# mit-acl/rl_collision_avoidance

Hardware: AMD Instinct MI355X
Metric: agent-steps/sec (env.step) at 4 agents x 8192 worlds per GPU (higher is better)
Workload: dtype f64

## Files before the change

__graft_entry__.py:

```python
import os
import sys

ROOT = os.path.dirname(os.path.abspath(__file__))
if ROOT not in sys.path:
    sys.path.insert(0, ROOT)


def build() -> None:
    from rl_collision_avoidance_amd import build as hip_build
    path = hip_build.build(verbose=True)
    assert os.path.exists(path)
    try:
        for kind in (1, 2, 3, 4):
            hip_build.build_ulp_fault(kind)
    except Exception as exc:
        print("warning: development variant not built (%s); the tests that need it build it themselves" % exc)
    try:
        hip_build.build_crowd_dev()
    except Exception as exc:
        print("warning: crowd development variant not built (%s); tests/test_gpu_crowd.py builds it itself" % exc)
    try:
        hip_build.build_plain_dist()
    except Exception as exc:
        print("warning: plain-distance development variant not built (%s); tests/test_gpu_relay_trim.py builds it itself" % exc)
    from oracle import c_oracle
    c_oracle.build()
    import rl_collision_avoidance_amd
    from rl_collision_avoidance_amd import _lib
    handle = _lib.lib()
    for name, _, _ in _lib.SYMBOLS:
        getattr(handle, name)
    print("build ok:", path)


def smoke() -> None:
    import numpy as np
    import torch
    from oracle import c_oracle as co
    from rl_collision_avoidance_amd.batched_env import BatchedCollisionAvoidanceEnv

    assert torch.cuda.is_available(), "smoke() needs cuda:0"
    W, N, seed = 256, 4, 17
    env = BatchedCollisionAvoidanceEnv(W, device="cuda:0", seed=seed)
    env.reset()
    ocfg, ogen = co.default_cfg(N), co.default_gen(N, N, pool_size=int(env.cfg.gen_pool_size))
    st = co.State.empty(W, N)
    ep = np.zeros(W, np.uint32)
    co.generate(ocfg, ogen, seed, st, ep)
    rng = np.random.default_rng(seed)
    for t in range(40):
        acts = rng.integers(0, 11, size=(W, N)).astype(np.int32)
        obs, rew, done, go = env.step_autoreset(torch.from_numpy(acts).cuda())
        oobs, orew, odone, ogo = co.step_autoreset(ocfg, ogen, seed, st, ep, acts)
        assert np.array_equal(done.cpu().numpy(), odone) and np.array_equal(go.cpu().numpy(), ogo)
        d = np.abs(obs.cpu().numpy() - oobs)
        d[..., 3] = np.minimum(d[..., 3], np.abs(d[..., 3] - 2 * np.pi))
        assert d.max() <= 1e-5
        assert np.abs(rew.cpu().numpy() - orew).max() <= 1e-5
    fl = env.get_state()[2].cpu().numpy().view(np.uint32)
    assert np.array_equal(fl, st.flags)
    acts16 = rng.integers(0, 11, size=(16, W, N)).astype(np.int32)
    slots = env.new_step_slots(16, packed=True)
    pk_all, go_all = env.step_autoreset_packed(torch.from_numpy(acts16).cuda(), slots)
    wdt = env.obs_width
    for k in range(16):
        oobs, orew, odone, ogo = co.step_autoreset(ocfg, ogen, seed, st, ep, acts16[k])
        pk = pk_all[k].cpu().numpy()
        d = np.abs(pk[..., :wdt] - oobs)
        d[..., 3] = np.minimum(d[..., 3], np.abs(d[..., 3] - 2 * np.pi))
        assert d.max() <= 1e-5 and np.abs(pk[..., wdt] - orew).max() <= 1e-5, k
        assert np.array_equal(pk[..., wdt + 1].astype(np.uint8), odone) and np.array_equal(go_all[k].cpu().numpy(), ogo), k
    assert np.array_equal(env.get_state()[2].cpu().numpy().view(np.uint32), st.flags)
    obs = torch.from_numpy(np.ascontiguousarray(pk[..., :wdt])).cuda()
    from rl_collision_avoidance_amd.ga3c.network import NetworkVP_rnn
    from rl_collision_avoidance_amd.ga3c.policy_kernel import FusedPolicy
    net = NetworkVP_rnn(env.config).to("cuda:0")
    view = obs.view(W * N, -1)[:, 1:]
# ... 44 lines not shown
```

rl_collision_avoidance_amd/build.py:

```python
from __future__ import annotations

import os
import shutil
import subprocess

PKG_DIR = os.path.dirname(os.path.abspath(__file__))
ROOT = os.path.dirname(PKG_DIR)
CSRC = os.path.join(PKG_DIR, "csrc")
LIB_PATH = os.path.join(PKG_DIR, "libcavoid_hip.so")
SOURCES = [os.path.join(CSRC, "cavoid_capi.hip"), os.path.join(CSRC, "cavoid_multistep.hip"), os.path.join(CSRC, "cavoid_rvo.hip"),
           os.path.join(CSRC, "cavoid_relay.hip"), os.path.join(CSRC, "cavoid_quad.hip"), os.path.join(CSRC, "cavoid_rollout_capi.hip"),
           os.path.join(CSRC, "cavoid_policy_capi.hip"), os.path.join(CSRC, "cavoid_comm_capi.hip"), os.path.join(CSRC, "cavoid_actor.hip"),
           os.path.join(CSRC, "cavoid_actor_rvo.hip"), os.path.join(CSRC, "cavoid_actor_frozen.hip"), os.path.join(CSRC, "cavoid_crowd.hip"),
           os.path.join(CSRC, "cavoid_policy_ws.hip"), os.path.join(CSRC, "cavoid_policy_train_ring.hip"),
           os.path.join(CSRC, "cavoid_policy_wsring.hip"), os.path.join(CSRC, "cavoid_crowd_push.hip"), os.path.join(CSRC, "cavoid_crowd_rvo.hip"),
           os.path.join(CSRC, "cavoid_crowd_actor.hip")]
HEADERS = {
    "cavoid_capi.hip": ["cavoid_kernels.hpp", "cavoid_launch.hpp", "cavoid_host.hpp", "cavoid_crowd.hpp", "cavoid_crowd_rvo.hpp"],
    "cavoid_multistep.hip": ["cavoid_kernels.hpp", "cavoid_launch.hpp", "cavoid_host.hpp"],
    "cavoid_rvo.hip": ["cavoid_kernels.hpp", "cavoid_launch.hpp", "cavoid_host.hpp"],
    "cavoid_relay.hip": ["cavoid_kernels.hpp", "cavoid_relay.hpp", "cavoid_launch.hpp", "cavoid_host.hpp"],
    "cavoid_quad.hip": ["cavoid_kernels.hpp", "cavoid_quad.hpp", "cavoid_launch.hpp", "cavoid_host.hpp"],
    "cavoid_rollout_capi.hip": ["cavoid_rollout.hpp", "cavoid_rollout_host.hpp", "cavoid_host.hpp"],
    "cavoid_policy_capi.hip": ["cavoid_policy.hpp", "cavoid_policy_split.hpp", "cavoid_policy_split8.hpp", "cavoid_policy_crowd.hpp", "cavoid_policy_host.hpp",
# ... 145 lines not shown
    out = variant_path("crowd2")
    if os.path.exists(out):
        return out
    build()
    objs = _compile_objects([], "", False, verbose)
    jobs, swap = [], {}
    for name in ("cavoid_capi.hip", "cavoid_multistep.hip", "cavoid_crowd.hip", "cavoid_crowd_rvo.hip"):
        src = os.path.join(CSRC, name)
        obj = os.path.join(OBJ_DIR, name.replace(".hip", ".crowd2.o"))
        jobs.append([hipcc()] + FLAGS + EXTRA_FLAGS.get(name, []) + ["-DCAVOID_DEV_CROWD_FROM_N=2", "-DCAVOID_DEV_ONLY_N", "-c", src, "-o", obj])
        swap[os.path.join(OBJ_DIR, name.replace(".hip", ".o"))] = obj
    if verbose:
        for j in jobs:
            print(" ".join(j), flush=True)
    with ThreadPoolExecutor(max_workers=len(jobs)) as pool:
        list(pool.map(subprocess.check_call, jobs))
    for old in glob.glob(os.path.join(FAULT_DIR, "libcavoid_hip_crowd2-*.so")):
        os.remove(old)
    tmp = out + ".tmp"
    _link([swap.get(o, o) for o in objs], tmp, verbose)
    os.replace(tmp, out)
    return out


def build_plain_dist(verbose: bool = False) -> str:
    import glob
    from concurrent.futures import ThreadPoolExecutor
    out = variant_path("plaindist")
    if os.path.exists(out):
        return out
    build()
    objs = _compile_objects([], "", False, verbose)
    jobs, swap = [], {}
    for name in ("cavoid_capi.hip", "cavoid_multistep.hip", "cavoid_rvo.hip", "cavoid_relay.hip"):
        src = os.path.join(CSRC, name)
        obj = os.path.join(OBJ_DIR, name.replace(".hip", ".plaindist.o"))
        jobs.append([hipcc()] + FLAGS + EXTRA_FLAGS.get(name, []) +
                    ["-DCAVOID_MIRROR_DIST=0", "-DCAVOID_RELAY_ROLE_ARGS=0", "-DCAVOID_DEV_ONLY_N", "-DCAVOID_DEV_ENV_NS=3,4,5,6,10",
                     "-DCAVOID_DEV_RELAY_NS=3,4,5,6", "-c", src, "-o", obj])
        swap[os.path.join(OBJ_DIR, name.replace(".hip", ".o"))] = obj
    if verbose:
        for j in jobs:
            print(" ".join(j), flush=True)
    with ThreadPoolExecutor(max_workers=len(jobs)) as pool:
        list(pool.map(subprocess.check_call, jobs))
    for old in glob.glob(os.path.join(FAULT_DIR, "libcavoid_hip_plaindist-*.so")):
        os.remove(old)
    tmp = out + ".tmp"
    _link([swap.get(o, o) for o in objs], tmp, verbose)
    os.replace(tmp, out)
    return out


if __name__ == "__main__":
    import sys
    if "--trace" in sys.argv:
        print(build_trace(verbose=True))
    elif "--plain-dist" in sys.argv:
        print(build_plain_dist(verbose=True))
    elif "--crowd-dev" in sys.argv:
        print(build_crowd_dev(verbose=True))
    elif "--ulp-faults" in sys.argv:
        for kind in (1, 2, 3, 4):
            print(build_ulp_fault(kind, verbose=True))
    else:
        print(build(force=True, verbose=True))
```

rl_collision_avoidance_amd/csrc/cavoid_kernels.hpp:

```cpp
#pragma once
#include <hip/hip_runtime.h>
#include <stdint.h>

#include "cavoid.h"

namespace cavoid {

#ifdef CAVOID_TRACE
__device__ unsigned long long *g_trace = nullptr;
#define CAVOID_STAMP(k)                                                                \
    do {                                                                               \
        if (lane == 0 && g_trace) g_trace[wave * 16 + (k)] = (unsigned long long)clock64(); \
    } while (0)
#else
#define CAVOID_STAMP(k) do { } while (0)
#endif

#define CAVOID_RARE(x) __builtin_expect(!!(x), 0)
#ifndef CAVOID_SKIP
#define CAVOID_SKIP 0
#endif

constexpr double kPi = 3.14159265358979323846;
constexpr int kTileMaxAgents = 16;
// ... 15 lines not shown
    int32_t max_other, width, sort_method, dynamics, actions_fp32, timeout_enabled, num_actions;
    int32_t gen_mode, rvo_enabled;
    uint32_t pool_epoch;
    int32_t pool_size;
    int32_t ahead;
    int32_t prefetch_pool;
    int32_t tile_rows;
    int32_t wpw;
    int32_t rvo_lds_floats;
    int32_t park_floats;
    int32_t evaluate_mode;
    int32_t stream_obs;
    uint32_t switches;
    uint32_t seed_lo, seed_hi;
    int64_t num_worlds, world_offset;
    const double *action_table;
};

enum : uint32_t {
    kSwSkipDonePairs = 1u,
    kSwExactGap = 2u,
    kSwIndexTie = 4u,
    kSwWrapClosed = 8u,
};
struct KState {
    double *px, *py, *heading, *t_rem;
    float *gx, *gy, *radius, *pref, *speed;
    uint32_t *flags;
    uint32_t *episode;
};

struct alignas(64) PoolRec {
    double px, py, heading, t_rem;
    float gx, gy, radius, pref;
    uint32_t flags;
    uint32_t pad[3];
};
static_assert(sizeof(PoolRec) == 64, "pool record must be one 64-byte line");

struct KIO {
    PoolRec *pool_out;
    const int32_t *actions;
    const float *cont;
    const uint8_t *mask;
    float *obs;
    float *rew;
    uint8_t *done;
    uint8_t *game_over;
    int64_t action_stride;
    int64_t out_step_stride;
    int32_t n_steps;
    int32_t obs_stride;
    int32_t packed;
    uint32_t *ahead_hi;
};

__device__ __forceinline__ double wrap_closed_fixup(double a, uint32_t switches) {
    if (CAVOID_RARE(switches & kSwWrapClosed)) a = a == -kPi ? kPi : a;
    return a;
}
__device__ __forceinline__ double wrap_angle(double a, uint32_t switches) {
    a = a >= kPi ? a - 2.0 * kPi : a;
    a = a < -kPi ? a + 2.0 * kPi : a;
    if (CAVOID_RARE(__ballot(a >= kPi || a < -kPi) != 0ull)) {
        while (a >= kPi) a -= 2.0 * kPi;
        while (a < -kPi) a += 2.0 * kPi;
    }
    return wrap_closed_fixup(a, switches);
}
__device__ __forceinline__ double wrap_once(double h, uint32_t switches) {
    h = h >= kPi ? h - 2.0 * kPi : h;
    h = h < -kPi ? h + 2.0 * kPi : h;
    return wrap_closed_fixup(h, switches);
}

__device__ __forceinline__ void wave_lds_sync() {
    __builtin_amdgcn_fence(__ATOMIC_RELEASE, "wavefront");
    __builtin_amdgcn_wave_barrier();
    __builtin_amdgcn_fence(__ATOMIC_ACQUIRE, "wavefront");
}

struct U4 { uint32_t x, y, z, w; };
__device__ __forceinline__ U4 philox4x32(uint32_t c0, uint32_t c1, uint32_t c2, uint32_t c3, uint32_t k0, uint32_t k1) {
#pragma unroll
    for (int r = 0; r < 10; ++r) {
        const uint64_t p0 = (uint64_t)0xD2511F53u * c0, p1 = (uint64_t)0xCD9E8D57u * c2;
        const uint32_t n0 = (uint32_t)(p1 >> 32) ^ c1 ^ k0, n1 = (uint32_t)p1;
        const uint32_t n2 = (uint32_t)(p0 >> 32) ^ c3 ^ k1, n3 = (uint32_t)p0;
        c0 = n0; c1 = n1; c2 = n2; c3 = n3;
        k0 += 0x9E3779B9u; k1 += 0xBB67AE85u;
    }
    return U4{c0, c1, c2, c3};
}
__device__ __forceinline__ double u01(uint32_t r) { return (double)(r >> 8) * (1.0 / 16777216.0); }

struct Agent {
    double px, py, heading, t_rem, vx, vy;
    float gx, gy, radius, pref, speed;
    uint32_t flags;
};

struct alignas(16) StageRec { double px, py; float vxf, vyf, r, pad; };
static_assert(sizeof(StageRec) == 32, "two 16-byte reads per neighbour");
constexpr int kRingDoubleFromN = 6;
__host__ __device__ constexpr int lds_floats_block() { return 64 * 2; }
__host__ __device__ constexpr int lds_floats_fixed(int n) { return (n >= kRingDoubleFromN ? 128 : 64) * (int)(sizeof(StageRec) / sizeof(float)); }
// ... 1491 lines not shown
```

rl_collision_avoidance_amd/csrc/cavoid_launch.hpp:

```cpp
#pragma once
#include <hip/hip_runtime.h>
#include <hip/hip_ext.h>

#include <type_traits>

#include "cavoid.h"
#include "cavoid_host.hpp"
#include "cavoid_kernels.hpp"

struct cavoid_env {
    int device = 0;
    int64_t W = 0, A = 0, world_offset = 0;
    cavoid_cfg cfg{};
    cavoid::KCfg k{};
    cavoid::KState st{};
    cavoid::PoolRec *pool = nullptr;
    uint32_t *pool_episode = nullptr;
    int64_t pool_size = 0;
    int ahead_R = 0;
    uint32_t *ahead_hi[2] = {nullptr, nullptr};
    int ahead_cur = 0;
    int ahead_budget = 0;
    bool ahead_primed = false;
    bool ahead_always = false;
    int64_t ahead_refills = 0;
    int relay_topup_nc = -1;
    size_t relay_topup_lds = 0;
    bool relay_topup_fits = false;
    void *slab = nullptr;
    void *pool_slab = nullptr;
    double *d_actions = nullptr;
    int waves_per_block = 4;
    int grid = 0;
    int pipeline = 2;
    int relay_consumers = 3;
    int latency_mode = 0;
    int quad = -1;
    int prefetch_single = 0;
    int last_form = CAVOID_FORM_NONE;
    int last_relay_consumers = 0;
    hipEvent_t ev0 = nullptr, ev1 = nullptr;
};


namespace cavoid {

template <int... Ns>
struct NList {};
#ifdef CAVOID_DEV_ONLY_N
#ifndef CAVOID_DEV_ENV_NS
#define CAVOID_DEV_ENV_NS 4, 10
#endif
#ifndef CAVOID_DEV_RELAY_NS
#define CAVOID_DEV_RELAY_NS 4
#endif
using EnvNs = NList<CAVOID_DEV_ENV_NS>;
using RelayNs = NList<CAVOID_DEV_RELAY_NS>;
using QuadNs = NList<4>;
#else
using EnvNs = NList<1, 2, 3, 4, 5, 6, 7, 8, 9, 10, 11, 12, 13, 14, 15, 16>;
using RelayNs = NList<1, 2, 3, 4, 5, 6>;
using QuadNs = NList<2, 3, 4, 5, 6, 10>;
#endif

#ifdef CAVOID_DEV_CROWD_FROM_N
constexpr int kCrowdFromN = CAVOID_DEV_CROWD_FROM_N;
#else
constexpr int kCrowdFromN = kTileMaxAgents + 1;
#endif
static inline bool crowd_form(int max_agents) { return max_agents >= kCrowdFromN; }

template <int... Ns, class F>
static inline int dispatch_n(int n, NList<Ns...>, F &&f) {
    int rc = CAVOID_EUNSUPPORTED;
    (void)((n == Ns ? (rc = f(std::integral_constant<int, Ns>{}), true) : false) || ...);
    return rc;
}

template <class K, class... Args>
static inline void launch_kernel(K kernel, dim3 grid, dim3 block, size_t lds, hipStream_t s, hipEvent_t ev_start, hipEvent_t ev_stop,
                                 const Args &...args) {
// ... 86 lines not shown
```

rl_collision_avoidance_amd/csrc/cavoid_relay.hip:

```cpp
#include "cavoid_launch.hpp"
#include "cavoid_relay.hpp"

using namespace cavoid;

constexpr int kRelayMaxDevices = 64;
template <int N>
static int relay_allow_lds() {
    static bool allowed[kRelayMaxDevices] = {};
    int dev = 0;
    HIP_TRY(hipGetDevice(&dev));
    const bool cached = dev >= 0 && dev < kRelayMaxDevices;
    if (cached && allowed[dev]) return CAVOID_OK;
    if (hipFuncSetAttribute(reinterpret_cast<const void *>(env_relay_kernel<N>), hipFuncAttributeMaxDynamicSharedMemorySize, (int)kRelayLdsLimit) != hipSuccess) {
        (void)hipGetLastError();
        return CAVOID_EUNSUPPORTED;
    }
    if (cached) allowed[dev] = true;
    return CAVOID_OK;
}

struct RelayShape {
    int nc = 0;
    size_t lds = 0;
    bool topup = false;
};
template <int N>
static int relay_shape_n(cavoid_env *e, int tile_floats, bool want_topup, RelayShape &sh) {
    int nc = e->relay_consumers;
    while (nc > 1 && relay_lds_fixed_bytes<N>() + (size_t)nc * tile_floats * sizeof(float) > kRelayLdsLimit) --nc;
    const size_t lds = relay_lds_fixed_bytes<N>() + (size_t)nc * tile_floats * sizeof(float);
    if (lds > kRelayLdsLimit || (nc < 2 && e->relay_consumers >= 2)) return CAVOID_EUNSUPPORTED;
    if (lds > 65536) {
        const int rc_opt = relay_allow_lds<N>();
        if (rc_opt != CAVOID_OK) return rc_opt;
    }
    sh.nc = nc;
    sh.lds = lds;
    sh.topup = false;
    if (want_topup && e->k.gen_mode == 0) {
        if (e->relay_topup_nc != nc || e->relay_topup_lds != lds) {
            int blocks = 0;
            if (hipOccupancyMaxActiveBlocksPerMultiprocessor(&blocks, reinterpret_cast<const void *>(env_relay_kernel<N>), 64 * (4 + nc), lds) != hipSuccess) {
                (void)hipGetLastError();
                blocks = 0;
            }
            e->relay_topup_nc = nc;
            e->relay_topup_lds = lds;
            e->relay_topup_fits = blocks >= 2;
        }
        sh.topup = e->relay_topup_fits;
    }
    return CAVOID_OK;
}
static int relay_shape(cavoid_env *e, const KIO &io, bool want_topup, RelayShape &sh) {
    const KCfg &k = e->k;
    if (k.rvo_enabled || k.pool_size <= 0 || !io.obs || !io.actions || io.cont) return CAVOID_EUNSUPPORTED;
    if (k.switches & kSwSkipDonePairs) return CAVOID_EUNSUPPORTED;
    const int64_t tiles = (e->W + k.wpw - 1) / k.wpw;
    if (tiles > 512) return CAVOID_EUNSUPPORTED;
    if (e->cfg.max_agents > kRelayMaxAgents) return CAVOID_EUNSUPPORTED;
    const int row = io.obs_stride;
    const int tile_floats = (k.tile_rows * row + 3) & ~3;
    if (k.tile_rows < k.wpw * e->cfg.max_agents) return CAVOID_EUNSUPPORTED;
    return dispatch_n(e->cfg.max_agents, RelayNs{}, [&](auto n) -> int { return relay_shape_n<decltype(n)::value>(e, tile_floats, want_topup, sh); });
}

static bool relay_wants_topup(const cavoid_env *e, hipStream_t s) {
    if (e->ahead_R <= 0 || e->ahead_always || e->k.gen_mode != 0) return false;
    hipStreamCaptureStatus cap = hipStreamCaptureStatusNone;
    (void)hipStreamIsCapturing(s, &cap);
    return cap == hipStreamCaptureStatusNone;
}

bool cavoid_relay_takes_topup(cavoid_env *e, const KIO &io, hipStream_t s) {
    RelayShape sh;
    return relay_wants_topup(e, s) && relay_shape(e, io, true, sh) == CAVOID_OK && sh.topup;
}

int cavoid_launch_relay(cavoid_env *e, const KIO &io, hipStream_t s, hipEvent_t ev_start, hipEvent_t ev_stop) {
    RelayShape sh;
    const int rc_shape = relay_shape(e, io, io.ahead_hi != nullptr, sh);
    if (rc_shape != CAVOID_OK) return rc_shape;
    if ((io.ahead_hi != nullptr) != sh.topup) return CAVOID_EINVAL;
    const int64_t tiles = (e->W + e->k.wpw - 1) / e->k.wpw;
    const dim3 grid((unsigned)tiles), block(64 * (3 + sh.nc + (sh.topup ? 1 : 0)));
    const int rc = dispatch_n(e->cfg.max_agents, RelayNs{}, [&](auto n) -> int {
        launch_kernel(env_relay_kernel<decltype(n)::value>, grid, block, sh.lds, s, ev_start, ev_stop, e->k, e->st, e->pool, io);
        return CAVOID_OK;
    });
    if (rc != CAVOID_OK) return rc;
    HIP_TRY(hipGetLastError());
    return note_form(e, CAVOID_OK, CAVOID_FORM_RELAY, sh.nc);
}

#ifdef CAVOID_TRACE
int cavoid_debug_trace_relay(unsigned long long *dev_ptr) { return set_trace(dev_ptr); }
#endif
```

rl_collision_avoidance_amd/csrc/cavoid_relay.hpp:

```cpp
#pragma once
#include <cstddef>
#include <type_traits>

#include "cavoid_kernels.hpp"

namespace cavoid {

constexpr int kRelayMaxAgents = 6;
template <int N>
__host__ __device__ constexpr int relay_ring() { return N <= 5 ? 8 : 4; }
constexpr size_t kRelayLdsLimit = 80 * 1024;
constexpr int kRelayActRing = 64;
constexpr int kRelayActAhead = 48;
constexpr int kRelayEvq = 8;
constexpr int kRelayTopupMaxN = 5;

struct RelaySeq {
    int spec;
    int stage;
    int res;
    int fin;
    int act;
    int ev;
    int nxt;
    int cons[kRelayMaxConsumers];
    int cfin[kRelayMaxConsumers];
    int coop[2];
    int kernarg[2];
    int tile_id;
};
static_assert(sizeof(RelaySeq) % 16 == 0, "the event queue behind it holds 64-bit masks; the tiles further on are read 16 bytes at a time");
struct RelayTent { double px[64], py[64], vx[64], vy[64], heading[64]; float r[64], gx[64], gy[64], pref[64]; uint32_t flags[64]; };
struct RelayRes { uint32_t flags[64], ctl[64]; float rew[64]; };
struct RelayNxt { double px[64], py[64], heading[64], t_rem[64]; float gx[64], gy[64], radius[64], pref[64]; uint32_t flags[64]; };
#ifndef CAVOID_RELAY_ORDER
#define CAVOID_RELAY_ORDER 0x6432150
#endif
#ifndef CAVOID_RELAY_PRIO_D
#define CAVOID_RELAY_PRIO_D 3
#endif
#ifndef CAVOID_RELAY_PRIO_P
#define CAVOID_RELAY_PRIO_P 3
#endif
#ifndef CAVOID_RELAY_PRIO_L
#define CAVOID_RELAY_PRIO_L 0
#endif
#ifndef CAVOID_RELAY_PRIO_C
#define CAVOID_RELAY_PRIO_C 1
#endif
#ifndef CAVOID_RELAY_PRIO_T
#define CAVOID_RELAY_PRIO_T 0
#endif
#ifndef CAVOID_RELAY_ABL
#define CAVOID_RELAY_ABL 0
#endif
__device__ __forceinline__ int relay_role_of(int wv, int NC) {
    if (NC == 3) return (int)(((unsigned)CAVOID_RELAY_ORDER >> (4 * wv)) & 15u);
    return wv;
}
constexpr int kRelayCoopWaves = 3;
constexpr int kRelayCoopFromN = 4;
template <int N>
struct RelayCoop {
    static constexpr int K = Others<N>::K;
    uint64_t key[K][64];
    uint32_t bits[K][64];
};
template <int N>
__host__ __device__ constexpr size_t relay_coop_bytes() { return N >= kRelayCoopFromN ? sizeof(RelayCoop<N>) : 0; }
template <int N>
__host__ __device__ constexpr size_t relay_lds_fixed_bytes() {
    return (size_t)lds_floats_block() * sizeof(float) + sizeof(RelaySeq) + kRelayActRing * 64 + relay_ring<N>() * (sizeof(RelayTent) + sizeof(RelayRes)) +
           sizeof(RelayNxt) + kRelayEvq * sizeof(unsigned long long) + relay_coop_bytes<N>();
}

#ifdef CAVOID_TRACE
#define RELAY_STAMP(k)                                                                                         \
    do {                                                                                                       \
        if (lane0 == 0 && g_trace && t == (n_steps >> 1)) g_trace[wave * 32 + (k)] = (unsigned long long)clock64(); \
    } while (0)
#define RELAY_MARK(k)                                                                                          \
    do {                                                                                                       \
        if (lane0 == 0 && g_trace) g_trace[wave * 32 + (k)] = (unsigned long long)clock64();                   \
    } while (0)
#else
#define RELAY_STAMP(k) do { } while (0)
#define RELAY_MARK(k) do { } while (0)
#endif

typedef __attribute__((address_space(3))) volatile int relay_lds_int;
__device__ __forceinline__ int relay_peek(const int *p) { return __builtin_amdgcn_readfirstlane(*(relay_lds_int *)p); }
__device__ __forceinline__ void relay_wait(const int *p, int v) {
    while (relay_peek(p) < v) __builtin_amdgcn_s_sleep(1);
    asm volatile("" ::: "memory");
}
constexpr int kRelayPollLimit = 1 << 24;
__device__ __forceinline__ void relay_wait_bounded(const int *p, int v) {
    int polls = 0;
    while (relay_peek(p) < v) {
        if (++polls > kRelayPollLimit) __builtin_trap();
        __builtin_amdgcn_s_sleep(1);
    }
    asm volatile("" ::: "memory");
}
__device__ __forceinline__ void relay_spin(const int *p, int v) {
    while (relay_peek(p) < v) { }
    asm volatile("" ::: "memory");
}
__device__ __forceinline__ int relay_peek_issue(const int *p) { return *(relay_lds_int *)p; }
__device__ __forceinline__ int relay_seen(int v) { return __builtin_amdgcn_readfirstlane(v); }
typedef __attribute__((address_space(3))) volatile uint32_t relay_lds_u32;
typedef __attribute__((address_space(3))) volatile double relay_lds_f64;
__device__ __forceinline__ void relay_post(int *p, int v) {
    asm volatile("" ::: "memory");
// ... 117 lines not shown
__device__ __forceinline__ void relay_coop_arrive(int *p, int lane) {
    asm volatile("" ::: "memory");
    if (lane == 0) __hip_atomic_fetch_add((__attribute__((address_space(3))) int *)p, 1, __ATOMIC_RELAXED, __HIP_MEMORY_SCOPE_WORKGROUP);
    asm volatile("" ::: "memory");
    int polls = 0;
    while (relay_peek(p) < kRelayCoopWaves) {
        if (++polls > kRelayPollLimit) __builtin_trap();
    }
    asm volatile("" ::: "memory");
}
template <int N, bool SW>
__device__ __forceinline__ void relay_pair_part(const KCfg &c, const Agent &a, const Ego &e, const bool present, const ArrayStage<N> &st, const int pw,
                                                const int lane, RelayCoop<N> &co, float (&gapf)[Others<N>::K], float (&feat)[Others<N>::K][kFeat]) {
    const double ri = (double)a.radius;
#pragma unroll
    for (int o = 0; o < N - 1; ++o) {
        if (o % kRelayCoopWaves != pw) continue;
        const OtherState q = st.other(o);
        const float rjf = q.r;
        const double rx = q.px - a.px, ry = q.py - a.py;
#if defined(CAVOID_DEV_ULP_FAULT) && CAVOID_DEV_ULP_FAULT == 1
        const double d = sqrt_dist2((double)((float)rx * (float)rx) + ry * ry);
#else
        const double d = sqrt_dist2(rx * rx + ry * ry);
#endif
        const bool other = present && (rjf >= 0.0f);
        const bool seen = other && !(d > c.horizon);
        const double gap_o = d - ri - (double)rjf;
#if defined(CAVOID_DEV_ULP_FAULT) && CAVOID_DEV_ULP_FAULT == 3
        uint32_t hi = kKeyBias - (uint32_t)(int)rintf((float)gap_o * 100.0f);
#else
        uint32_t hi = kKeyBias - (uint32_t)(int)rint(gap_o * 100.0);
#endif
        uint32_t lo = orderable((float)(ry * e.tx - rx * e.ty));
        if (SW) {
            if (c.switches & kSwIndexTie) lo = (uint32_t)other_index(st.i, o, N);
            if (c.switches & kSwExactGap) { lo = 0u; hi = 0x7FFFFFFEu - (orderable((float)gap_o) >> 1); }
        }
        hi = seen ? hi : kKeySentinel + (uint32_t)o;
        co.key[o][lane] = ((uint64_t)hi << 32) | lo;
        co.bits[o][lane] = seen ? 2u : 0u;
        gapf[o] = (float)gap_o;
        neighbour_features(e, (float)e.prll_x, (float)e.prll_y, rx, ry, q, feat[o]);
    }
}

struct RelayArgs { KCfg c; KState s; const PoolRec *pool; KIO io; };
static_assert(alignof(KCfg) == 8 && alignof(KState) == 8 && alignof(KIO) == 8 && alignof(RelayArgs) == 8, "kernel arguments: 8-byte aligned");
static_assert(sizeof(KCfg) % 8 == 0 && sizeof(KState) % 8 == 0 && sizeof(KIO) % 8 == 0, "kernel arguments: whole 8-byte words, no tail padding to skip");
static_assert(offsetof(RelayArgs, c) == 0 && offsetof(RelayArgs, s) == sizeof(KCfg) && offsetof(RelayArgs, pool) == sizeof(KCfg) + sizeof(KState) &&
                  offsetof(RelayArgs, io) == sizeof(KCfg) + sizeof(KState) + sizeof(const PoolRec *) &&
                  sizeof(RelayArgs) == sizeof(KCfg) + sizeof(KState) + sizeof(const PoolRec *) + sizeof(KIO),
              "RelayArgs must be the kernel's argument segment, argument by argument");
static_assert(sizeof(KIO) == 104 && offsetof(KIO, n_steps) == 80 && offsetof(KIO, ahead_hi) == 96, "KIO changed: check what relay_coop_last reads from it");
template <class T>
__device__ __forceinline__ void relay_load_args(T &dst, const __attribute__((address_space(4))) T *src) {
    static_assert(sizeof(T) % 4 == 0, "whole words");
    const __attribute__((address_space(4))) uint32_t *w = (const __attribute__((address_space(4))) uint32_t *)src;
    uint32_t d[sizeof(T) / 4];
#pragma unroll
    for (int k = 0; k < (int)(sizeof(T) / 4); ++k) d[k] = w[k];
    __builtin_memcpy(&dst, d, sizeof(T));
}
#ifndef CAVOID_RELAY_ROLE_ARGS
#define CAVOID_RELAY_ROLE_ARGS 1
#endif
typedef const __attribute__((address_space(4))) RelayArgs *RelayArgP;
#if CAVOID_RELAY_ROLE_ARGS
#define RELAY_ROLE_ARGS_LOAD()                                                                         \
    unsigned long long kp_ = (unsigned long long)__builtin_amdgcn_kernarg_segment_ptr();               \
    asm volatile("" : "+s"(kp_));                                                                      \
    KCfg c; KState s; const PoolRec *pool; KIO io;                                                     \
    relay_load_args(s, &((RelayArgP)kp_)->s); relay_load_args(io, &((RelayArgP)kp_)->io);               \
    relay_load_args(c, &((RelayArgP)kp_)->c); relay_load_args(pool, &((RelayArgP)kp_)->pool);            \
    asm volatile("" : "+s"(c.wpw), "+s"(c.num_worlds))
#define RELAY_ROLE_PIN(...) asm volatile("" : __VA_ARGS__)
#define RELAY_ROLE_STATE(name)                                                                         \
    unsigned long long kps_ = (unsigned long long)__builtin_amdgcn_kernarg_segment_ptr();              \
    asm volatile("" : "+s"(kps_));                                                                     \
    KState name;                                                                                       \
    relay_load_args(name, &((RelayArgP)kps_)->s)
#else
#define RELAY_ROLE_ARGS_LOAD() const KCfg &c = c_; const KState &s = s_; const PoolRec *const pool = pool_; const KIO &io = io_
#define RELAY_ROLE_STATE(name) const KState &name = s_
#define RELAY_ROLE_PIN(...) do { } while (0)
#endif
#define RELAY_ROLE_ARGS()                                                                              \
    RELAY_ROLE_ARGS_LOAD();                                                                            \
    (void)s; (void)pool;                                                                               \
    [[maybe_unused]] const int ostride = io.obs_stride;                                                \
    [[maybe_unused]] const int tile_floats = (c.tile_rows * ostride + 3) & ~3;                         \
    const int wpw = c.wpw, lanes_used = wpw * N;                                                       \
    [[maybe_unused]] const int64_t wave = blockIdx.x;                      \
    const int64_t w0 = wave * wpw;                                                                     \
    const int lw = lane0 / N;                                                                          \
    [[maybe_unused]] const int i0 = lane0 - lw * N;                                                    \
    [[maybe_unused]] const int64_t w = w0 + lw;                                                        \
    [[maybe_unused]] const bool active = lane0 < lanes_used && w < c.num_worlds;                       \
    [[maybe_unused]] const int base0 = lane0 < lanes_used ? lw * N : 0;                                \
    [[maybe_unused]] const int64_t a_idx0 = w * N + i0;                                                \
    [[maybe_unused]] const bool packed = io.packed != 0;                                               \
    [[maybe_unused]] int64_t worlds_here = c.num_worlds - w0;                                          \
    if (worlds_here > wpw) worlds_here = wpw;                                                          \
    if (worlds_here < 0) worlds_here = 0;                                                              \
    [[maybe_unused]] const int n_steps = io.n_steps
template <int N>
__device__ __forceinline__ void relay_coop_last(unsigned char *smem) {
    unsigned char *sp = smem + lds_floats_block() * sizeof(float);
    RelaySeq *seq = reinterpret_cast<RelaySeq *>(sp); sp += sizeof(RelaySeq) + kRelayEvq * sizeof(unsigned long long);
    const unsigned long long kp = (unsigned long long)(uint32_t)relay_peek(&seq->kernarg[0]) | ((unsigned long long)(uint32_t)relay_peek(&seq->kernarg[1]) << 32);
    typedef const __attribute__((address_space(4))) RelayArgs *ArgP;
    const ArgP ka = (ArgP)kp;
    KCfg c;
    KIO io;
    relay_load_args(c, &ka->c);
    relay_load_args(io, &ka->io);
    RelayTent *tents = reinterpret_cast<RelayTent *>(sp); sp += relay_ring<N>() * sizeof(RelayTent) + sizeof(RelayNxt);
    RelayRes *ress = reinterpret_cast<RelayRes *>(sp); sp += relay_ring<N>() * sizeof(RelayRes) + kRelayActRing * 64;
    RelayCoop<N> *coopb = reinterpret_cast<RelayCoop<N> *>(sp); sp += relay_coop_bytes<N>();
    float *tiles = reinterpret_cast<float *>(sp);
    const int lane0 = threadIdx.x & 63;
    const int tile_nc = relay_peek(&seq->tile_id);
    const int NC = tile_nc >> 16;
    const int role = relay_role_of(threadIdx.x >> 6, NC);
    const int pw = role < 2 ? role : 2;
    const int ostride = io.obs_stride;
    const int tile_floats = (c.tile_rows * ostride + 3) & ~3;
    const int wpw = c.wpw, lanes_used = wpw * N;
    const int64_t wave = tile_nc & 0xFFFF;
    const int64_t w0 = wave * wpw;
    const int lw = lane0 / N, i0 = lane0 - lw * N;
    const int64_t w = w0 + lw;
    const bool active = lane0 < lanes_used && w < c.num_worlds;
    const int base0 = lane0 < lanes_used ? lw * N : 0;
    const int64_t a_idx0 = w * N + i0;
    const bool packed = io.packed != 0;
    int64_t worlds_here = c.num_worlds - w0;
    if (worlds_here > wpw) worlds_here = wpw;
    if (worlds_here < 0) worlds_here = 0;
    const int n_steps = io.n_steps;
    constexpr int K = Others<N>::K;
    const int t = n_steps - 1;
    const int cid_l = t % NC;
    float *tile = tiles + (size_t)cid_l * tile_floats;
    RelayCoop<N> &co = *coopb;
    relay_wait_bounded(&seq->fin, t + 1);
    const RelayTent &f = tents[t & (relay_ring<N>() - 1)];
    const RelayRes &v = ress[t & (relay_ring<N>() - 1)];
    Agent ao;
    ao.px = f.px[lane0]; ao.py = f.py[lane0]; ao.vx = f.vx[lane0]; ao.vy = f.vy[lane0];
    ao.heading = f.heading[lane0]; ao.t_rem = 0.0;
    ao.gx = f.gx[lane0]; ao.gy = f.gy[lane0]; ao.speed = 0.0f;
    ao.radius = f.r[lane0]; ao.pref = f.pref[lane0]; ao.flags = v.flags[lane0];
    const uint32_t ctl_c = v.ctl[lane0];
    const float rew_c = v.rew[lane0], done_c = (ctl_c & 1u) ? 1.0f : 0.0f;
    const bool present = active && (ao.flags & CAVOID_F_PRESENT);
    const Ego e = ego_frame_obs(c, ao);
    const ArrayStage<N> as{f.px, f.py, f.vx, f.vy, f.r, i0, base0};
    float gapf[K], feat[K][kFeat];
#pragma unroll
    for (int o = 0; o < K; ++o) {
        gapf[o] = 0.0f;
#pragma unroll
        for (int q = 0; q < kFeat; ++q) feat[o][q] = 0.0f;
    }
    if (c.switches != 0u) relay_pair_part<N, true>(c, ao, e, present, as, pw, lane0, co, gapf, feat);
    else relay_pair_part<N, false>(c, ao, e, present, as, pw, lane0, co, gapf, feat);
    relay_coop_arrive(&seq->coop[0], lane0);
    Key key[K];
    uint32_t valid = 0u;
    if (N == 1) key[0].set(kKeySentinel, 0u);
#pragma unroll
    for (int o = 0; o < N - 1; ++o) {
        key[o].v = co.key[o][lane0];
        valid |= (co.bits[o][lane0] & 2u) ? (1u << o) : 0u;
    }
    if (t - NC >= 0) relay_wait_bounded(&seq->cons[cid_l], t - NC + 1);
    const int rows_active = (int)worlds_here * N;
    assemble_obs<N, false, true, ArrayStage<N>, NoHook, false, PartOthers>(c, ao, e, active, lane0, as, key, gapf, feat, valid, tile, nullptr,
                                                                           rows_active, ostride, false, 0.0f, 0.0f, wave, NoHook(), false, nullptr,
                                                                           PartOthers{pw, kRelayCoopWaves});
    if (pw == 0 && active && lane0 < rows_active) {
        const int M = c.max_other;
        const int m = __popc(valid);
        const int first = m > M ? m - M : 0;
        const int kept = m - first;
        write_row_head(tile + lane0 * ostride, ao, e, present, kept, kept, M, packed, c.width, rew_c, done_c);
    }
    relay_coop_arrive(&seq->coop[1], lane0);
    if (io.out_step_stride == 0)
        for (int o = 0; o < NC; ++o) relay_wait_bounded(&seq->cfin[o], 1);
    const int64_t slot_w = (int64_t)t * io.out_step_stride;
    if (worlds_here > 0) {
        float *dst = io.obs + (slot_w + w0) * N * ostride;
        const bool lines = ((rows_active * ostride) & 31) == 0 && (reinterpret_cast<uintptr_t>(dst) & 127) == 0;
        if (io.out_step_stride != 0 && lines) flush_tile<4, true, true>(tile, dst, rows_active * ostride, pw * 64 + lane0, 64 * kRelayCoopWaves);
        else if (io.out_step_stride != 0) flush_tile<4, true>(tile, dst, rows_active * ostride, pw * 64 + lane0, 64 * kRelayCoopWaves);
        else flush_tile<4>(tile, dst, rows_active * ostride, pw * 64 + lane0, 64 * kRelayCoopWaves);
    }
    if (pw == 0 && active) {
        if (!packed) {
            io.rew[slot_w * N + a_idx0] = rew_c;
            io.done[slot_w * N + a_idx0] = (ctl_c & 1u) ? 1 : 0;
        }
        if (i0 == 0) io.game_over[slot_w + w] = (ctl_c & 2u) ? 1 : 0;
    }
    if (pw == 0) RELAY_MARK(29);
}

template <int N>
__device__ __forceinline__ void relay_topup() {
    __builtin_amdgcn_s_setprio(CAVOID_RELAY_PRIO_T);
    unsigned long long kp = (unsigned long long)__builtin_amdgcn_kernarg_segment_ptr();
    asm volatile("" : "+s"(kp));
    typedef const __attribute__((address_space(4))) RelayArgs *ArgP;
    const ArgP ka = (ArgP)kp;
    KCfg c;
    uint32_t *episode, *hi;
    const PoolRec *ring;
    relay_load_args(c, &ka->c);
    relay_load_args(episode, &ka->s.episode);
    relay_load_args(ring, &ka->pool);
    relay_load_args(hi, &ka->io.ahead_hi);
    const int lane0 = threadIdx.x & 63;
    const int wpw = c.wpw, lanes_used = wpw * N;
    const int lw = lane0 / N, i0 = lane0 - lw * N;
    const int64_t w = (int64_t)blockIdx.x * wpw + lw;
    const bool active = lane0 < lanes_used && w < c.num_worlds;
    const int base0 = lane0 < lanes_used ? lw * N : 0;
    uint32_t ep = 0u, fh = 0u;
    if (active) {
        ep = episode[w];
        fh = hi[w];
    }
    asm volatile("" : "+v"(ep), "+v"(fh));
    __syncthreads();
    ahead_fill_range<N, true>(c, ep, fh, active, w, i0, base0, lane0, hi, const_cast<PoolRec *>(ring), c.ahead, 0, 1, nullptr, nullptr);
}

template <int N>
__global__ void __launch_bounds__(64 * (4 + kRelayMaxConsumers), N <= kRelayTopupMaxN ? 4 : 1) env_relay_kernel(const KCfg c_, const KState s_, const PoolRec *pool_, const KIO io_) {
    extern __shared__ __attribute__((aligned(16))) unsigned char smem[];
    unsigned char *sp = smem;
    double *lds_tab = reinterpret_cast<double *>(sp); sp += lds_floats_block() * sizeof(float);
    RelaySeq *seq = reinterpret_cast<RelaySeq *>(sp); sp += sizeof(RelaySeq);
    unsigned long long *evq = reinterpret_cast<unsigned long long *>(sp); sp += kRelayEvq * sizeof(unsigned long long);
    RelayTent *tents = reinterpret_cast<RelayTent *>(sp); sp += relay_ring<N>() * sizeof(RelayTent);
    RelayNxt *nbuf = reinterpret_cast<RelayNxt *>(sp); sp += sizeof(RelayNxt);
    RelayRes *ress = reinterpret_cast<RelayRes *>(sp); sp += relay_ring<N>() * sizeof(RelayRes);
    unsigned char *actring = sp; sp += kRelayActRing * 64;
    RelayCoop<N> *coopb = reinterpret_cast<RelayCoop<N> *>(sp); sp += relay_coop_bytes<N>();
    float *tiles = reinterpret_cast<float *>(sp);

    const int NC = (blockDim.x >> 6) - 3 - (io_.ahead_hi ? 1 : 0);
    const int role = relay_role_of(threadIdx.x >> 6, NC);
    const int lane0 = threadIdx.x & 63;
    constexpr bool kCoop = N >= kRelayCoopFromN;
    const bool coop_role = role < 2 || role == 2 + NC;

    if (role == 0 && lane0 < (int)(sizeof(RelaySeq) / sizeof(int))) reinterpret_cast<int *>(seq)[lane0] = 0;
// ... 397 lines not shown
```

Before: 25.13 billion.

## Give relay tail step a dedicated LDS tile handled by one wave

For small agent counts (N<=4) with per-step output slots, the last step's observation assembly gets an extra LDS tile when it fits. A single wave then does the full pair pass and writes that step alone, instead of the three-wave cooperative path that waits on consumer tiles. The aim is to shorten the tail of the multistep relay launch by skipping cooperative barriers and the wait for a free consumer tile. It costs extra LDS and an occupancy check to confirm two blocks still fit, and it adds a development build with the tail path disabled for comparison.

After: 25.57 billion (median of 6 runs). Within noise of the previous version (+1.8%).

```diff
diff --git a/__graft_entry__.py b/__graft_entry__.py
--- a/__graft_entry__.py
+++ b/__graft_entry__.py
@@ -23,6 +23,10 @@
         hip_build.build_plain_dist()
     except Exception as exc:
         print("warning: plain-distance development variant not built (%s); tests/test_gpu_relay_trim.py builds it itself" % exc)
+    try:
+        hip_build.build_plain_tail()
+    except Exception as exc:
+        print("warning: plain-tail development variant not built (%s); tests/test_gpu_relay_tail.py builds it itself" % exc)
     from oracle import c_oracle
     c_oracle.build()
     import rl_collision_avoidance_amd
diff --git a/rl_collision_avoidance_amd/build.py b/rl_collision_avoidance_amd/build.py
--- a/rl_collision_avoidance_amd/build.py
+++ b/rl_collision_avoidance_amd/build.py
@@ -221,12 +221,36 @@
     return out
 
 
+def build_plain_tail(verbose: bool = False) -> str:
+    import glob
+    out = variant_path("plaintail")
+    if os.path.exists(out):
+        return out
+    build()
+    objs = _compile_objects([], "", False, verbose)
+    name = "cavoid_relay.hip"
+    obj = os.path.join(OBJ_DIR, name.replace(".hip", ".plaintail.o"))
+    cmd = [hipcc()] + FLAGS + EXTRA_FLAGS.get(name, []) + ["-DCAVOID_RELAY_TAIL=0", "-DCAVOID_DEV_ONLY_N", "-DCAVOID_DEV_RELAY_NS=3,4,5,6",
+                                                          "-c", os.path.join(CSRC, name), "-o", obj]
+    if verbose:
+        print(" ".join(cmd), flush=True)
+    subprocess.check_call(cmd)
+    for old in glob.glob(os.path.join(FAULT_DIR, "libcavoid_hip_plaintail-*.so")):
+        os.remove(old)
+    tmp = out + ".tmp"
+    _link([obj if o == os.path.join(OBJ_DIR, name.replace(".hip", ".o")) else o for o in objs], tmp, verbose)
+    os.replace(tmp, out)
+    return out
+
+
 if __name__ == "__main__":
     import sys
     if "--trace" in sys.argv:
         print(build_trace(verbose=True))
     elif "--plain-dist" in sys.argv:
         print(build_plain_dist(verbose=True))
+    elif "--plain-tail" in sys.argv:
+        print(build_plain_tail(verbose=True))
     elif "--crowd-dev" in sys.argv:
         print(build_crowd_dev(verbose=True))
     elif "--ulp-faults" in sys.argv:
diff --git a/rl_collision_avoidance_amd/csrc/cavoid_kernels.hpp b/rl_collision_avoidance_amd/csrc/cavoid_kernels.hpp
--- a/rl_collision_avoidance_amd/csrc/cavoid_kernels.hpp
+++ b/rl_collision_avoidance_amd/csrc/cavoid_kernels.hpp
@@ -91,6 +91,7 @@
     int32_t n_steps;
     int32_t obs_stride;
     int32_t packed;
+    int32_t relay_extra;
     uint32_t *ahead_hi;
 };
 
diff --git a/rl_collision_avoidance_amd/csrc/cavoid_launch.hpp b/rl_collision_avoidance_amd/csrc/cavoid_launch.hpp
--- a/rl_collision_avoidance_amd/csrc/cavoid_launch.hpp
+++ b/rl_collision_avoidance_amd/csrc/cavoid_launch.hpp
@@ -24,9 +24,11 @@
     bool ahead_primed = false;
     bool ahead_always = false;
     int64_t ahead_refills = 0;
-    int relay_topup_nc = -1;
-    size_t relay_topup_lds = 0;
-    bool relay_topup_fits = false;
+    struct relay_occ_t {
+        int threads = -1;
+        size_t lds = 0;
+        bool fits = false;
+    } relay_occ[2];
     void *slab = nullptr;
     void *pool_slab = nullptr;
     double *d_actions = nullptr;
diff --git a/rl_collision_avoidance_amd/csrc/cavoid_relay.hip b/rl_collision_avoidance_amd/csrc/cavoid_relay.hip
--- a/rl_collision_avoidance_amd/csrc/cavoid_relay.hip
+++ b/rl_collision_avoidance_amd/csrc/cavoid_relay.hip
@@ -21,35 +21,51 @@
 
 struct RelayShape {
     int nc = 0;
+    int extra = 0;
     size_t lds = 0;
     bool topup = false;
 };
 template <int N>
-static int relay_shape_n(cavoid_env *e, int tile_floats, bool want_topup, RelayShape &sh) {
+static bool relay_two_resident(cavoid_env *e, int which, int threads, size_t lds) {
+    cavoid_env::relay_occ_t &o = e->relay_occ[which];
+    if (o.threads != threads || o.lds != lds) {
+        int blocks = 0;
+        if (hipOccupancyMaxActiveBlocksPerMultiprocessor(&blocks, reinterpret_cast<const void *>(env_relay_kernel<N>), threads, lds) != hipSuccess) {
+            (void)hipGetLastError();
+            blocks = 0;
+        }
+        o.threads = threads;
+        o.lds = lds;
+        o.fits = blocks >= 2;
+    }
+    return o.fits;
+}
+template <int N>
+static int relay_shape_n(cavoid_env *e, int tile_floats, bool want_topup, bool own_rows, RelayShape &sh) {
     int nc = e->relay_consumers;
-    while (nc > 1 && relay_lds_fixed_bytes<N>() + (size_t)nc * tile_floats * sizeof(float) > kRelayLdsLimit) --nc;
-    const size_t lds = relay_lds_fixed_bytes<N>() + (size_t)nc * tile_floats * sizeof(float);
+    const size_t tile_bytes = (size_t)tile_floats * sizeof(float);
+    while (nc > 1 && relay_lds_fixed_bytes<N>() + (size_t)nc * tile_bytes > kRelayLdsLimit) --nc;
+    const size_t lds = relay_lds_fixed_bytes<N>() + (size_t)nc * tile_bytes;
     if (lds > kRelayLdsLimit || (nc < 2 && e->relay_consumers >= 2)) return CAVOID_EUNSUPPORTED;
-    if (lds > 65536) {
+    int extra = 0;
+#if CAVOID_RELAY_TAIL
+    if (N >= kRelayCoopFromN && N <= kRelayAloneMaxN && own_rows)
+        while (extra < kRelayMaxExtraTiles && lds + (size_t)(extra + 1) * tile_bytes <= kRelayLdsLimit) ++extra;
+#else
+    (void)own_rows;
+#endif
+    if (lds + (size_t)extra * tile_bytes > 65536) {
         const int rc_opt = relay_allow_lds<N>();
-        if (rc_opt != CAVOID_OK) return rc_opt;
+        if (rc_opt != CAVOID_OK) {
+            if (lds > 65536) return rc_opt;
+            extra = 0;
+        }
     }
     sh.nc = nc;
-    sh.lds = lds;
-    sh.topup = false;
-    if (want_topup && e->k.gen_mode == 0) {
-        if (e->relay_topup_nc != nc || e->relay_topup_lds != lds) {
-            int blocks = 0;
-            if (hipOccupancyMaxActiveBlocksPerMultiprocessor(&blocks, reinterpret_cast<const void *>(env_relay_kernel<N>), 64 * (4 + nc), lds) != hipSuccess) {
-                (void)hipGetLastError();
-                blocks = 0;
-            }
-            e->relay_topup_nc = nc;
-            e->relay_topup_lds = lds;
-            e->relay_topup_fits = blocks >= 2;
-        }
-        sh.topup = e->relay_topup_fits;
-    }
+    sh.topup = want_topup && e->k.gen_mode == 0 && relay_two_resident<N>(e, 0, 64 * (4 + nc), lds);
+    if (extra > 0 && !relay_two_resident<N>(e, 1, 64 * (3 + nc + (sh.topup ? 1 : 0)), lds + (size_t)extra * tile_bytes)) extra = 0;
+    sh.extra = extra;
+    sh.lds = lds + (size_t)extra * tile_bytes;
     return CAVOID_OK;
 }
 static int relay_shape(cavoid_env *e, const KIO &io, bool want_topup, RelayShape &sh) {
@@ -62,7 +78,7 @@
     const int row = io.obs_stride;
     const int tile_floats = (k.tile_rows * row + 3) & ~3;
     if (k.tile_rows < k.wpw * e->cfg.max_agents) return CAVOID_EUNSUPPORTED;
-    return dispatch_n(e->cfg.max_agents, RelayNs{}, [&](auto n) -> int { return relay_shape_n<decltype(n)::value>(e, tile_floats, want_topup, sh); });
+    return dispatch_n(e->cfg.max_agents, RelayNs{}, [&](auto n) -> int { return relay_shape_n<decltype(n)::value>(e, tile_floats, want_topup, io.out_step_stride != 0, sh); });
 }
 
 static bool relay_wants_topup(const cavoid_env *e, hipStream_t s) {
@@ -84,8 +100,10 @@
     if ((io.ahead_hi != nullptr) != sh.topup) return CAVOID_EINVAL;
     const int64_t tiles = (e->W + e->k.wpw - 1) / e->k.wpw;
     const dim3 grid((unsigned)tiles), block(64 * (3 + sh.nc + (sh.topup ? 1 : 0)));
+    KIO kio = io;
+    kio.relay_extra = sh.extra;
     const int rc = dispatch_n(e->cfg.max_agents, RelayNs{}, [&](auto n) -> int {
-        launch_kernel(env_relay_kernel<decltype(n)::value>, grid, block, sh.lds, s, ev_start, ev_stop, e->k, e->st, e->pool, io);
+        launch_kernel(env_relay_kernel<decltype(n)::value>, grid, block, sh.lds, s, ev_start, ev_stop, e->k, e->st, e->pool, kio);
         return CAVOID_OK;
     });
     if (rc != CAVOID_OK) return rc;
diff --git a/rl_collision_avoidance_amd/csrc/cavoid_relay.hpp b/rl_collision_avoidance_amd/csrc/cavoid_relay.hpp
--- a/rl_collision_avoidance_amd/csrc/cavoid_relay.hpp
+++ b/rl_collision_avoidance_amd/csrc/cavoid_relay.hpp
@@ -60,6 +60,11 @@
 }
 constexpr int kRelayCoopWaves = 3;
 constexpr int kRelayCoopFromN = 4;
+#ifndef CAVOID_RELAY_TAIL
+#define CAVOID_RELAY_TAIL 1
+#endif
+constexpr int kRelayMaxExtraTiles = 1;
+constexpr int kRelayAloneMaxN = 4;
 template <int N>
 struct RelayCoop {
     static constexpr int K = Others<N>::K;
@@ -283,7 +288,8 @@
                   offsetof(RelayArgs, io) == sizeof(KCfg) + sizeof(KState) + sizeof(const PoolRec *) &&
                   sizeof(RelayArgs) == sizeof(KCfg) + sizeof(KState) + sizeof(const PoolRec *) + sizeof(KIO),
               "RelayArgs must be the kernel's argument segment, argument by argument");
-static_assert(sizeof(KIO) == 104 && offsetof(KIO, n_steps) == 80 && offsetof(KIO, ahead_hi) == 96, "KIO changed: check what relay_coop_last reads from it");
+static_assert(sizeof(KIO) == 104 && offsetof(KIO, n_steps) == 80 && offsetof(KIO, relay_extra) == 92 && offsetof(KIO, ahead_hi) == 96,
+              "KIO changed: check what relay_coop_last reads from it");
 template <class T>
 __device__ __forceinline__ void relay_load_args(T &dst, const __attribute__((address_space(4))) T *src) {
     static_assert(sizeof(T) % 4 == 0, "whole words");
@@ -372,9 +378,49 @@
     const int n_steps = io.n_steps;
     constexpr int K = Others<N>::K;
     const int t = n_steps - 1;
+#if CAVOID_RELAY_TAIL
+    if (N <= kRelayAloneMaxN && io.relay_extra > 0) {
+        if (pw != 1) return;
+        RELAY_MARK(4);
+        float *tile = tiles + (size_t)NC * tile_floats;
+        relay_wait_bounded(&seq->fin, t + 1);
+        const RelayTent &f = tents[t & (relay_ring<N>() - 1)];
+        const RelayRes &v = ress[t & (relay_ring<N>() - 1)];
+        Agent ao;
+        ao.px = f.px[lane0]; ao.py = f.py[lane0]; ao.vx = f.vx[lane0]; ao.vy = f.vy[lane0];
+        ao.heading = f.heading[lane0]; ao.t_rem = 0.0;
+        ao.gx = f.gx[lane0]; ao.gy = f.gy[lane0]; ao.speed = 0.0f;
+        ao.radius = f.r[lane0]; ao.pref = f.pref[lane0]; ao.flags = v.flags[lane0];
+        const uint32_t ctl_c = v.ctl[lane0];
+        const float rew_c = v.rew[lane0], done_c = (ctl_c & 1u) ? 1.0f : 0.0f;
+        const bool present = active && (ao.flags & CAVOID_F_PRESENT);
+        const Ego e = ego_frame_obs(c, ao);
+        Key key[K];
+        float gapf[K];
+        uint32_t valid;
+        bool hit;
+        double min_gap;
+        const ArrayStage<N> as{f.px, f.py, f.vx, f.vy, f.r, i0, base0};
+        float feat[K][kFeat];
+        pair_pass<N, false, true>(c, ao, e, present, as, key, gapf, feat, valid, hit, min_gap);
+        const int64_t slot_w = (int64_t)t * io.out_step_stride;
+        assemble_obs<N, false, true, ArrayStage<N>>(c, ao, e, active, lane0, as, key, gapf, feat, valid, tile, io.obs + (slot_w + w0) * N * ostride,
+                                                    (int)worlds_here * N, ostride, packed, rew_c, done_c, wave, NoHook(), true);
+        if (active) {
+            if (!packed) {
+                io.rew[slot_w * N + a_idx0] = rew_c;
+                io.done[slot_w * N + a_idx0] = (ctl_c & 1u) ? 1 : 0;
+            }
+            if (i0 == 0) io.game_over[slot_w + w] = (ctl_c & 2u) ? 1 : 0;
+        }
+        RELAY_MARK(29);
+        return;
+    }
+#endif
     const int cid_l = t % NC;
     float *tile = tiles + (size_t)cid_l * tile_floats;
     RelayCoop<N> &co = *coopb;
+    RELAY_MARK(pw == 0 ? 6 : pw == 1 ? 4 : 5);
     relay_wait_bounded(&seq->fin, t + 1);
     const RelayTent &f = tents[t & (relay_ring<N>() - 1)];
     const RelayRes &v = ress[t & (relay_ring<N>() - 1)];
@@ -398,6 +444,7 @@
     if (c.switches != 0u) relay_pair_part<N, true>(c, ao, e, present, as, pw, lane0, co, gapf, feat);
     else relay_pair_part<N, false>(c, ao, e, present, as, pw, lane0, co, gapf, feat);
     relay_coop_arrive(&seq->coop[0], lane0);
+    if (pw == 0) RELAY_MARK(7);
     Key key[K];
     uint32_t valid = 0u;
     if (N == 1) key[0].set(kKeySentinel, 0u);
@@ -419,6 +466,7 @@
         write_row_head(tile + lane0 * ostride, ao, e, present, kept, kept, M, packed, c.width, rew_c, done_c);
     }
     relay_coop_arrive(&seq->coop[1], lane0);
+    if (pw == 0) RELAY_MARK(14);
     if (io.out_step_stride == 0)
         for (int o = 0; o < NC; ++o) relay_wait_bounded(&seq->cfin[o], 1);
     const int64_t slot_w = (int64_t)t * io.out_step_stride;
@@ -437,6 +485,7 @@
         if (i0 == 0) io.game_over[slot_w + w] = (ctl_c & 2u) ? 1 : 0;
     }
     if (pw == 0) RELAY_MARK(29);
+    if (pw == 1) RELAY_MARK(15);
 }
 
 template <int N>
```
